# rizar/attention-lvcsr

Hardware: AMD Instinct MI355X
Metric: encoder+attention+decoder training frames/sec (whole node) (higher is better)
Workload: dtype f32; 1 GPU; wsj_base: B=16 utterances x T=800 frames x F=40 fbank per GPU, L=100 labels; 256x256x256x256 BiGRU subsample [1, 1, 2, 2], content_and_conv attention, 256-unit GRU decoder; global_batch=16, per_gpu_batch=16, ragged=False, parallelism=dp1, optimizer=clip100+adadelta+maxnorm1, hip_graph=True, priming_steps=2, encoder_kernels=persistent clusters, full=False

## Files before the change

attention-lvcsr_amd/csrc/gemm.hip:

```cpp
#include "common.h"
#include "lvsr_hip.h"
#include "graph_cache.h"

#define BM 64
#define BN 64
#define BK 16
#define LDS_LD (BM + 4)

struct GemmArgs {
    const float* A; const float* B; float* C; const float* bias;
    int M, N, K, lda, ldb, ldc, transA, transB;
    float alpha, beta;
    int ksplit;
    int kchunk;
    float* part;
    int batch;
    long long sA, sB, sC;
};

__global__ __launch_bounds__(256) void lvsr_sgemm_kernel(GemmArgs g) {
    __shared__ float As[BK][LDS_LD];
    __shared__ float Bs[BK][LDS_LD];
    const int tid = threadIdx.x, lane = tid & 63, wave = tid >> 6;
    const int m0 = blockIdx.y * BM, n0 = blockIdx.x * BN;
    int zsplit = blockIdx.z;
    if (g.batch > 1) {
        g.A += blockIdx.z * g.sA; g.B += blockIdx.z * g.sB; g.C += blockIdx.z * g.sC;
        zsplit = 0;
    }
    const int kbeg = zsplit * g.kchunk;
    const int kend = min(g.K, kbeg + g.kchunk);
    const int rowbase = (wave >> 1) * 32, colbase = (wave & 1) * 32;
    f32x4 acc[2][2];
#pragma unroll
    for (int i = 0; i < 2; ++i)
#pragma unroll
        for (int j = 0; j < 2; ++j) acc[i][j] = (f32x4){0.f, 0.f, 0.f, 0.f};

    for (int k0 = kbeg; k0 < kend; k0 += BK) {
        if (!g.transA) {
            const int kk = tid & 15, mm = tid >> 4;
#pragma unroll
            for (int p = 0; p < 4; ++p) {
                const int m = m0 + mm + p * 16, k = k0 + kk;
                As[kk][mm + p * 16] = (m < g.M && k < kend) ? g.A[(size_t)m * g.lda + k] : 0.f;
            }
        } else {
            const int mm = tid & 63, kk = tid >> 6;
#pragma unroll
            for (int p = 0; p < 4; ++p) {
                const int m = m0 + mm, k = k0 + kk + p * 4;
                As[kk + p * 4][mm] = (m < g.M && k < kend) ? g.A[(size_t)k * g.lda + m] : 0.f;
            }
        }
        if (!g.transB) {
            const int nn = tid & 63, kk = tid >> 6;
#pragma unroll
            for (int p = 0; p < 4; ++p) {
                const int n = n0 + nn, k = k0 + kk + p * 4;
                Bs[kk + p * 4][nn] = (n < g.N && k < kend) ? g.B[(size_t)k * g.ldb + n] : 0.f;
            }
        } else {
            const int kk = tid & 15, nn = tid >> 4;
#pragma unroll
            for (int p = 0; p < 4; ++p) {
                const int n = n0 + nn + p * 16, k = k0 + kk;
                Bs[kk][nn + p * 16] = (n < g.N && k < kend) ? g.B[(size_t)n * g.ldb + k] : 0.f;
            }
        }
        __syncthreads();
#pragma unroll
        for (int ks = 0; ks < BK; ks += 4) {
            const int kr = ks + (lane >> 4), li = lane & 15;
            float a[2], b[2];
            a[0] = As[kr][rowbase + li];
            a[1] = As[kr][rowbase + 16 + li];
            b[0] = Bs[kr][colbase + li];
            b[1] = Bs[kr][colbase + 16 + li];
#pragma unroll
            for (int i = 0; i < 2; ++i)
#pragma unroll
                for (int j = 0; j < 2; ++j)
                    acc[i][j] = __builtin_amdgcn_mfma_f32_16x16x4f32(a[i], b[j], acc[i][j], 0, 0, 0);
        }
        __syncthreads();
    }
#pragma unroll
    for (int i = 0; i < 2; ++i)
#pragma unroll
        for (int j = 0; j < 2; ++j)
#pragma unroll
            for (int r = 0; r < 4; ++r) {
                const int m = m0 + rowbase + i * 16 + (lane >> 4) * 4 + r;
                const int n = n0 + colbase + j * 16 + (lane & 15);
                if (m < g.M && n < g.N) {
                    if (g.ksplit > 1) {
                        g.part[((size_t)zsplit * g.M + m) * g.N + n] = acc[i][j][r];
                    } else {
                        float v = g.alpha * acc[i][j][r];
                        if (g.beta != 0.f) v += g.beta * g.C[(size_t)m * g.ldc + n];
                        if (g.bias) v += g.bias[n];
                        g.C[(size_t)m * g.ldc + n] = v;
                    }
                }
            }
}

typedef float f32x16 __attribute__((ext_vector_type(16)));
#define GM 128
#define GN 128
#define GK 32
#define GLD 36

template <bool CONTIG_K, int TX, bool GUARD>
__device__ __forceinline__ void gemm2_tile_load(const float* __restrict__ p, int ld, int x0, int X, int k0, int kend, bool vec,
                                                float4 (&r)[TX / 32]) {
    if (CONTIG_K) {
#pragma unroll
        for (int h = 0; h < TX / 32; ++h) {
            const int u = threadIdx.x + h * 256;
            const int x = x0 + (u >> 3), k = k0 + (u & 7) * 4;
            if (!GUARD) r[h] = *(const float4*)(p + (size_t)x * ld + k);
            else r[h] = (x < X && k < kend) ? ld4g(p + (size_t)x * ld + k, kend - k, vec) : make_float4(0.f, 0.f, 0.f, 0.f);
        }
    } else {
        const int k = k0 + (threadIdx.x >> 6) * 8 + (threadIdx.x & 7);
#pragma unroll
        for (int h = 0; h < TX / 32; ++h) {
            const int x = x0 + 4 * (h * 8 + ((threadIdx.x >> 3) & 7));
            if (!GUARD) r[h] = *(const float4*)(p + (size_t)k * ld + x);
            else r[h] = (k < kend && x < X) ? ld4g(p + (size_t)k * ld + x, X - x, vec) : make_float4(0.f, 0.f, 0.f, 0.f);
        }
    }
}
__device__ __forceinline__ int gemm2_col(int k) { return (k & ~7) + ((k & 1) << 2) + ((k & 7) >> 1); }

template <bool CONTIG_K, int TX>
__device__ __forceinline__ void gemm2_tile_store(float (*S)[GLD], const float4 (&r)[TX / 32]) {
    if (CONTIG_K) {
#pragma unroll
        for (int h = 0; h < TX / 32; ++h) {
            const int u = threadIdx.x + h * 256;
            const int c0 = ((u & 7) >> 1) * 8 + (u & 1) * 2;
            *(float2*)&S[u >> 3][c0] = make_float2(r[h].x, r[h].z);
            *(float2*)&S[u >> 3][c0 + 4] = make_float2(r[h].y, r[h].w);
        }
    } else {
        const int k = gemm2_col((threadIdx.x >> 6) * 8 + (threadIdx.x & 7));
#pragma unroll
        for (int h = 0; h < TX / 32; ++h) {
            const int x = 4 * (h * 8 + ((threadIdx.x >> 3) & 7));
            S[x][k] = r[h].x; S[x + 1][k] = r[h].y; S[x + 2][k] = r[h].z; S[x + 3][k] = r[h].w;
        }
    }
}

__device__ __forceinline__ int gemm_xcd_order(int L, int total) {
    const int xcd = L & 7, per = total >> 3, rem = total & 7;
    return xcd * per + min(xcd, rem) + (L >> 3);
}

template <int TM, int TN, bool TA, bool TB, bool FAST>
__device__ __forceinline__ void sgemm_tile(GemmArgs g, int bx, int by, int bz) {
    constexpr int MI = TM / 64, NI = TN / 64;
    __shared__ __attribute__((aligned(16))) float As[2][TM][GLD];
    __shared__ __attribute__((aligned(16))) float Bs[2][TN][GLD];
    const int lane = threadIdx.x & 63, wave = threadIdx.x >> 6;
    if (g.batch > 1) {
        g.A += bz * g.sA; g.B += bz * g.sB; g.C += bz * g.sC;
        bz = 0;
    }
    const int m0 = by * TM, n0 = bx * TN;
    const int kbeg = bz * g.kchunk, kend = min(g.K, kbeg + g.kchunk);
    const int wm = (wave >> 1) * (TM / 2), wn = (wave & 1) * (TN / 2);
    const bool vecA = ((g.lda & 3) == 0) && ((((size_t)g.A) & 15) == 0);
    const bool vecB = ((g.ldb & 3) == 0) && ((((size_t)g.B) & 15) == 0);
    f32x16 acc[MI][NI];
#pragma unroll
    for (int i = 0; i < MI; ++i)
#pragma unroll
        for (int j = 0; j < NI; ++j)
#pragma unroll
            for (int r = 0; r < 16; ++r) acc[i][j][r] = 0.f;
    float4 ra[TM / 32], rb[TN / 32];
    const bool inside = FAST && m0 + TM <= g.M && n0 + TN <= g.N;
    if (inside && kbeg + GK <= kend) {
        gemm2_tile_load<!TA, TM, false>(g.A, g.lda, m0, g.M, kbeg, kend, true, ra);
        gemm2_tile_load<TB, TN, false>(g.B, g.ldb, n0, g.N, kbeg, kend, true, rb);
    } else {
        gemm2_tile_load<!TA, TM, true>(g.A, g.lda, m0, g.M, kbeg, kend, vecA, ra);
        gemm2_tile_load<TB, TN, true>(g.B, g.ldb, n0, g.N, kbeg, kend, vecB, rb);
    }
    gemm2_tile_store<!TA, TM>(As[0], ra);
    gemm2_tile_store<TB, TN>(Bs[0], rb);
    __syncthreads();
    int cur = 0;
    const int li = lane & 31, kh = (lane >> 5) * 4;
    for (int k0 = kbeg; k0 < kend; k0 += GK) {
        const bool more = k0 + GK < kend;
        float4 pa[2][MI], pb[2][NI];
#pragma unroll
        for (int i = 0; i < MI; ++i) pa[0][i] = *(const float4*)&As[cur][wm + 32 * i + li][kh];
#pragma unroll
        for (int j = 0; j < NI; ++j) pb[0][j] = *(const float4*)&Bs[cur][wn + 32 * j + li][kh];
#pragma unroll
        for (int q = 0; q < 4; ++q) {
            const int c = q & 1, n = c ^ 1;
            if (q + 1 < 4) {
#pragma unroll
                for (int i = 0; i < MI; ++i) pa[n][i] = *(const float4*)&As[cur][wm + 32 * i + li][kh + 8 * (q + 1)];
#pragma unroll
                for (int j = 0; j < NI; ++j) pb[n][j] = *(const float4*)&Bs[cur][wn + 32 * j + li][kh + 8 * (q + 1)];
            }
            __builtin_amdgcn_sched_barrier(0);
#pragma unroll
            for (int e = 0; e < 4; ++e)
#pragma unroll
                for (int i = 0; i < MI; ++i)
#pragma unroll
                    for (int j = 0; j < NI; ++j) {
                        const float x = e == 0 ? pa[c][i].x : e == 1 ? pa[c][i].y : e == 2 ? pa[c][i].z : pa[c][i].w;
                        const float y = e == 0 ? pb[c][j].x : e == 1 ? pb[c][j].y : e == 2 ? pb[c][j].z : pb[c][j].w;
                        acc[i][j] = __builtin_amdgcn_mfma_f32_32x32x2f32(x, y, acc[i][j], 0, 0, 0);
                    }
            __builtin_amdgcn_sched_barrier(0);
        }
        if (more) {
            if (inside && k0 + 2 * GK <= kend) {
                gemm2_tile_load<!TA, TM, false>(g.A, g.lda, m0, g.M, k0 + GK, kend, true, ra);
                gemm2_tile_load<TB, TN, false>(g.B, g.ldb, n0, g.N, k0 + GK, kend, true, rb);
            } else {
                gemm2_tile_load<!TA, TM, true>(g.A, g.lda, m0, g.M, k0 + GK, kend, vecA, ra);
                gemm2_tile_load<TB, TN, true>(g.B, g.ldb, n0, g.N, k0 + GK, kend, vecB, rb);
            }
            gemm2_tile_store<!TA, TM>(As[cur ^ 1], ra);
            gemm2_tile_store<TB, TN>(Bs[cur ^ 1], rb);
        }
        __syncthreads();
        cur ^= 1;
    }
#pragma unroll
    for (int i = 0; i < MI; ++i)
#pragma unroll
        for (int j = 0; j < NI; ++j)
#pragma unroll
            for (int r = 0; r < 16; ++r) {
                const int m = m0 + wm + i * 32 + (r & 3) + 8 * (r >> 2) + 4 * (lane >> 5);
                const int n = n0 + wn + j * 32 + (lane & 31);
                if (m < g.M && n < g.N) {
                    if (g.ksplit > 1) {
                        g.part[((size_t)bz * g.M + m) * g.N + n] = acc[i][j][r];
                    } else {
                        float v = g.alpha * acc[i][j][r];
                        if (g.beta != 0.f) v += g.beta * g.C[(size_t)m * g.ldc + n];
                        if (g.bias) v += g.bias[n];
                        g.C[(size_t)m * g.ldc + n] = v;
                    }
                }
            }
}
#define GU (GK / 8)
template <bool CONTIG_K, int TX>
__device__ __forceinline__ void gemm1_tile_load(const float* __restrict__ p, int ld, int x0, int X, int k0, int kend, bool vec,
                                               float4 (&r)[TX / 32]) {
#pragma unroll
    for (int h = 0; h < TX / 32; ++h) {
        const int u = threadIdx.x + h * 256;
        float4 v = make_float4(0.f, 0.f, 0.f, 0.f);
        if (CONTIG_K) {
            const int x = x0 + (u % TX), k = k0 + (u / TX) * 4;
            if (x < X && k < kend) v = ld4g(p + (size_t)x * ld + k, kend - k, vec);
        } else {
            const int k = k0 + u / (TX / 4), x = x0 + (u % (TX / 4)) * 4;
            if (k < kend && x < X) v = ld4g(p + (size_t)k * ld + x, X - x, vec);
        }
        r[h] = v;
    }
}
template <bool CONTIG_K, int TX>
__device__ __forceinline__ void gemm1_tile_load_fast(const float* __restrict__ p, int ld, int x0, int k0, float4 (&r)[TX / 32]) {
#pragma unroll
    for (int h = 0; h < TX / 32; ++h) {
        const int u = threadIdx.x + h * 256;
        if (CONTIG_K) r[h] = *(const float4*)(p + (size_t)(x0 + (u % TX)) * ld + k0 + (u / TX) * 4);
        else r[h] = *(const float4*)(p + (size_t)(k0 + u / (TX / 4)) * ld + x0 + (u % (TX / 4)) * 4);
    }
}
template <bool CONTIG_K, int TX>
__device__ __forceinline__ void gemm1_tile_store(float (*S)[TX + 4], const float4 (&r)[TX / 32]) {
#pragma unroll
    for (int h = 0; h < TX / 32; ++h) {
        const int u = threadIdx.x + h * 256;
        if (CONTIG_K) {
            const int x = u % TX, k = (u / TX) * 4;
            S[k + 0][x] = r[h].x; S[k + 1][x] = r[h].y; S[k + 2][x] = r[h].z; S[k + 3][x] = r[h].w;
        } else {
            const int k = u / (TX / 4), x = (u % (TX / 4)) * 4;
            *(float4*)&S[k][x] = r[h];
        }
    }
}

template <int TM, int TN, bool TA, bool TB, bool FAST>
__device__ __forceinline__ void sgemm_tile_kmajor(GemmArgs g, int bx, int by, int bz) {
    constexpr int MI = TM / 64, NI = TN / 64;
    __shared__ __attribute__((aligned(16))) float As[2][GK][TM + 4];
    __shared__ __attribute__((aligned(16))) float Bs[2][GK][TN + 4];
    const int lane = threadIdx.x & 63, wave = threadIdx.x >> 6;
    if (g.batch > 1) {
        g.A += bz * g.sA; g.B += bz * g.sB; g.C += bz * g.sC;
        bz = 0;
    }
    const int m0 = by * TM, n0 = bx * TN;
    const int kbeg = bz * g.kchunk, kend = min(g.K, kbeg + g.kchunk);
    const int wm = (wave >> 1) * (TM / 2), wn = (wave & 1) * (TN / 2);
    const bool vecA = ((g.lda & 3) == 0) && ((((size_t)g.A) & 15) == 0);
    const bool vecB = ((g.ldb & 3) == 0) && ((((size_t)g.B) & 15) == 0);
    f32x16 acc[MI][NI];
#pragma unroll
    for (int i = 0; i < MI; ++i)
#pragma unroll
        for (int j = 0; j < NI; ++j)
#pragma unroll
            for (int r = 0; r < 16; ++r) acc[i][j][r] = 0.f;
    float4 ra[TM / 32], rb[TN / 32];
    const bool inside = FAST && m0 + TM <= g.M && n0 + TN <= g.N;
    if (inside && kbeg + GK <= kend) {
        gemm1_tile_load_fast<!TA, TM>(g.A, g.lda, m0, kbeg, ra);
        gemm1_tile_load_fast<TB, TN>(g.B, g.ldb, n0, kbeg, rb);
    } else {
        gemm1_tile_load<!TA, TM>(g.A, g.lda, m0, g.M, kbeg, kend, vecA, ra);
        gemm1_tile_load<TB, TN>(g.B, g.ldb, n0, g.N, kbeg, kend, vecB, rb);
    }
    gemm1_tile_store<!TA, TM>(As[0], ra);
    gemm1_tile_store<TB, TN>(Bs[0], rb);
    __syncthreads();
    int cur = 0;
    for (int k0 = kbeg; k0 < kend; k0 += GK) {
        const bool more = k0 + GK < kend;
        if (more) {
            if (inside && k0 + 2 * GK <= kend) {
                gemm1_tile_load_fast<!TA, TM>(g.A, g.lda, m0, k0 + GK, ra);
                gemm1_tile_load_fast<TB, TN>(g.B, g.ldb, n0, k0 + GK, rb);
            } else {
                gemm1_tile_load<!TA, TM>(g.A, g.lda, m0, g.M, k0 + GK, kend, vecA, ra);
                gemm1_tile_load<TB, TN>(g.B, g.ldb, n0, g.N, k0 + GK, kend, vecB, rb);
            }
        }
        const int kr0 = lane >> 5, li = lane & 31;
        float pa[2][MI], pb[2][NI];
#pragma unroll
        for (int i = 0; i < MI; ++i) pa[0][i] = As[cur][kr0][wm + 32 * i + li];
#pragma unroll
        for (int j = 0; j < NI; ++j) pb[0][j] = Bs[cur][kr0][wn + 32 * j + li];
#pragma unroll
        for (int s = 0; s < GK / 2; ++s) {
            const int c = s & 1, n = c ^ 1;
            if (s + 1 < GK / 2) {
                const int kr = 2 * (s + 1) + kr0;
#pragma unroll
                for (int i = 0; i < MI; ++i) pa[n][i] = As[cur][kr][wm + 32 * i + li];
#pragma unroll
                for (int j = 0; j < NI; ++j) pb[n][j] = Bs[cur][kr][wn + 32 * j + li];
            }
            __builtin_amdgcn_sched_barrier(0);
#pragma unroll
            for (int i = 0; i < MI; ++i)
#pragma unroll
                for (int j = 0; j < NI; ++j)
                    acc[i][j] = __builtin_amdgcn_mfma_f32_32x32x2f32(pa[c][i], pb[c][j], acc[i][j], 0, 0, 0);
            __builtin_amdgcn_sched_barrier(0);
        }
        if (more) {
            gemm1_tile_store<!TA, TM>(As[cur ^ 1], ra);
            gemm1_tile_store<TB, TN>(Bs[cur ^ 1], rb);
        }
        __syncthreads();
        cur ^= 1;
    }
#pragma unroll
    for (int i = 0; i < MI; ++i)
#pragma unroll
        for (int j = 0; j < NI; ++j)
#pragma unroll
            for (int r = 0; r < 16; ++r) {
                const int m = m0 + wm + i * 32 + (r & 3) + 8 * (r >> 2) + 4 * (lane >> 5);
                const int n = n0 + wn + j * 32 + (lane & 31);
                if (m < g.M && n < g.N) {
                    if (g.ksplit > 1) {
                        g.part[((size_t)bz * g.M + m) * g.N + n] = acc[i][j][r];
                    } else {
                        float v = g.alpha * acc[i][j][r];
                        if (g.beta != 0.f) v += g.beta * g.C[(size_t)m * g.ldc + n];
                        if (g.bias) v += g.bias[n];
                        g.C[(size_t)m * g.ldc + n] = v;
                    }
                }
            }
}
template <bool TA, bool TB, bool FAST>
__device__ __forceinline__ void sgemm128_tile(GemmArgs g, int bx, int by, int bz) { sgemm_tile<128, 128, TA, TB, FAST>(g, bx, by, bz); }

template <bool TA, bool TB, bool FAST>
__global__ __launch_bounds__(256) void lvsr_sgemm64_kernel(GemmArgs g) {
    const int total = gridDim.x * gridDim.y * gridDim.z;
    const int t = gemm_xcd_order(blockIdx.x + gridDim.x * (blockIdx.y + gridDim.y * blockIdx.z), total);
    sgemm_tile_kmajor<64, 64, TA, TB, FAST>(g, t % gridDim.x, (t / gridDim.x) % gridDim.y, t / (gridDim.x * gridDim.y));
}

template <bool TA, bool TB, bool FAST>
__global__ __launch_bounds__(256) void lvsr_sgemm128_kernel(GemmArgs g) {
    const int total = gridDim.x * gridDim.y * gridDim.z;
    const int t = gemm_xcd_order(blockIdx.x + gridDim.x * (blockIdx.y + gridDim.y * blockIdx.z), total);
    sgemm128_tile<TA, TB, FAST>(g, t % gridDim.x, (t / gridDim.x) % gridDim.y, t / (gridDim.x * gridDim.y));
}

#define GROUP_MAX 40
struct GroupDesc {
    const float* A; const float* B; float* C;
    int M, N, K, lda, ldb, ldc;
    float beta;
    int ksplit, kchunk, gx, gy, unit0;
    long long part_off;
};
struct GroupPack { GroupDesc d[GROUP_MAX]; int n, total; float* part; };

template <bool FAST>
__global__ __launch_bounds__(256) void lvsr_sgemm128_grouped_tn_kernel(GroupPack pk) {
    const int t = gemm_xcd_order(blockIdx.x, pk.total);
    int p = 0;
    for (int x = 1; x < pk.n; ++x)
        if (t >= pk.d[x].unit0) p = x;
    const GroupDesc& d = pk.d[p];
    const int local = t - d.unit0;
    GemmArgs g;
    g.A = d.A; g.B = d.B; g.C = d.C; g.bias = nullptr;
    g.M = d.M; g.N = d.N; g.K = d.K; g.lda = d.lda; g.ldb = d.ldb; g.ldc = d.ldc; g.transA = 1; g.transB = 0;
    g.alpha = 1.f; g.beta = d.beta; g.ksplit = d.ksplit; g.kchunk = d.kchunk; g.part = pk.part + d.part_off;
    g.batch = 1; g.sA = g.sB = g.sC = 0;
    sgemm128_tile<true, false, FAST>(g, local % d.gx, (local / d.gx) % d.gy, local / (d.gx * d.gy));
}

__global__ __launch_bounds__(256) void lvsr_sgemm_grouped_reduce(GroupPack pk) {
    const GroupDesc& d = pk.d[blockIdx.y];
    if (d.ksplit <= 1) return;
    const size_t total = (size_t)d.M * d.N;
    const float* part = pk.part + d.part_off;
    for (size_t idx = (size_t)blockIdx.x * 256 + threadIdx.x; idx < total; idx += (size_t)gridDim.x * 256) {
        const int m = (int)(idx / d.N), n = (int)(idx % d.N);
        float s = 0.f;
        for (int z = 0; z < d.ksplit; ++z) s += part[(size_t)z * total + idx];
        if (d.beta != 0.f) s += d.beta * d.C[(size_t)m * d.ldc + n];
        d.C[(size_t)m * d.ldc + n] = s;
    }
}

__global__ __launch_bounds__(256) void lvsr_sgemm_splitk_reduce(GemmArgs g) {
    const size_t total = (size_t)g.M * g.N;
    for (size_t idx = (size_t)blockIdx.x * blockDim.x + threadIdx.x; idx < total; idx += (size_t)gridDim.x * blockDim.x) {
        const int m = (int)(idx / g.N), n = (int)(idx % g.N);
        float s = 0.f;
        for (int z = 0; z < g.ksplit; ++z) s += g.part[(size_t)z * total + idx];
        float v = g.alpha * s;
        if (g.beta != 0.f) v += g.beta * g.C[(size_t)m * g.ldc + n];
        if (g.bias) v += g.bias[n];
        g.C[(size_t)m * g.ldc + n] = v;
    }
}

__global__ __launch_bounds__(256) void lvsr_colsum_kernel(const float* X, int M, int N, int ldx, float* out, float beta,
                                                          int rows_per, float* part) {
    __shared__ float red[4][64];
    const int n = blockIdx.x * 64 + (threadIdx.x & 63);
    const int g = threadIdx.x >> 6;
    const int m0 = blockIdx.y * rows_per, m1 = min(M, m0 + rows_per);
    float s0 = 0.f, s1 = 0.f, s2 = 0.f, s3 = 0.f;
    if (n < N) {
        int m = m0 + g;
        for (; m + 12 < m1; m += 16) {
            s0 += X[(size_t)m * ldx + n];
            s1 += X[(size_t)(m + 4) * ldx + n];
            s2 += X[(size_t)(m + 8) * ldx + n];
            s3 += X[(size_t)(m + 12) * ldx + n];
        }
        for (; m < m1; m += 4) s0 += X[(size_t)m * ldx + n];
    }
    red[g][threadIdx.x & 63] = (s0 + s1) + (s2 + s3);
    __syncthreads();
    if (g == 0 && n < N) {
        const int c = threadIdx.x & 63;
        const float v = ((red[0][c] + red[1][c]) + red[2][c]) + red[3][c];
        if (part) part[(size_t)blockIdx.y * N + n] = v;
        else out[n] = (beta != 0.f ? beta * out[n] : 0.f) + v;
    }
}

#define COLSUM_MANY_MAX 32
struct ColsumMember { const float* X; float* out; float* part; int M, N, ldx, S, rows_per, nx, block0, fin0; float beta; };
struct ColsumPack { ColsumMember m[COLSUM_MANY_MAX]; int n; };
__global__ __launch_bounds__(256) void lvsr_colsum_many_kernel(ColsumPack pk) {
    __shared__ float red[4][64];
    int p = 0;
    for (int i = 1; i < pk.n; ++i)
        if ((int)blockIdx.x >= pk.m[i].block0) p = i;
    const ColsumMember& c = pk.m[p];
    const int local = blockIdx.x - c.block0, bx = local % c.nx, by = local / c.nx;
    const int n = bx * 64 + (threadIdx.x & 63);
    const int g = threadIdx.x >> 6;
    const int m0 = by * c.rows_per, m1 = min(c.M, m0 + c.rows_per);
    const float* X = c.X;
    const int ldx = c.ldx;
    float s0 = 0.f, s1 = 0.f, s2 = 0.f, s3 = 0.f;
    if (n < c.N) {
        int m = m0 + g;
        for (; m + 12 < m1; m += 16) {
            s0 += X[(size_t)m * ldx + n];
            s1 += X[(size_t)(m + 4) * ldx + n];
            s2 += X[(size_t)(m + 8) * ldx + n];
            s3 += X[(size_t)(m + 12) * ldx + n];
        }
        for (; m < m1; m += 4) s0 += X[(size_t)m * ldx + n];
    }
    red[g][threadIdx.x & 63] = (s0 + s1) + (s2 + s3);
    __syncthreads();
    if (g == 0 && n < c.N) {
        const int col = threadIdx.x & 63;
        const float v = ((red[0][col] + red[1][col]) + red[2][col]) + red[3][col];
        if (c.S > 1) c.part[(size_t)by * c.N + n] = v;
        else c.out[n] = (c.beta != 0.f ? c.beta * c.out[n] : 0.f) + v;
    }
}
__global__ __launch_bounds__(256) void lvsr_colsum_many_finish(ColsumPack pk) {
    int p = 0;
    for (int i = 1; i < pk.n; ++i)
        if ((int)blockIdx.x >= pk.m[i].fin0) p = i;
    const ColsumMember& c = pk.m[p];
    if (c.S <= 1) return;
    const int n = ((int)blockIdx.x - c.fin0) * 256 + threadIdx.x;
    if (n >= c.N) return;
    float v = 0.f;
    for (int s = 0; s < c.S; ++s) v += c.part[(size_t)s * c.N + n];
    c.out[n] = (c.beta != 0.f ? c.beta * c.out[n] : 0.f) + v;
}

__global__ __launch_bounds__(256) void lvsr_colsum_finish(const float* part, int S, int N, float* out, float beta) {
    const int n = blockIdx.x * 256 + threadIdx.x;
    if (n >= N) return;
    float v = 0.f;
    for (int s = 0; s < S; ++s) v += part[(size_t)s * N + n];
    out[n] = (beta != 0.f ? beta * out[n] : 0.f) + v;
}

#define COPY_MANY_MAX 32
struct CopyPack { lvsr_copy_desc d[COPY_MANY_MAX]; int n; };
__global__ __launch_bounds__(256) void lvsr_copy2d_many_kernel(CopyPack pk) {
    const lvsr_copy_desc& d = pk.d[blockIdx.y];
    const bool vec = ((d.cols | d.lds | d.ldd) & 3) == 0 && ((((size_t)d.src) | ((size_t)d.dst)) & 15) == 0;
    if (d.rows == 1) {
        for (int c = blockIdx.x * 256 + threadIdx.x; c < d.cols; c += gridDim.x * 256)
            d.dst[c] = d.beta != 0.f ? d.src[c] + d.beta * d.dst[c] : d.src[c];
        return;
    }
    for (int r = blockIdx.x; r < d.rows; r += gridDim.x) {
        const float* s = d.src + (size_t)r * d.lds;
        float* o = d.dst + (size_t)r * d.ldd;
        if (d.beta != 0.f) {
            for (int c = threadIdx.x; c < d.cols; c += 256) o[c] = s[c] + d.beta * o[c];
        } else if (vec) {
            for (int c = threadIdx.x * 4; c < d.cols; c += 1024) *(float4*)(o + c) = *(const float4*)(s + c);
        } else {
            for (int c = threadIdx.x; c < d.cols; c += 256) o[c] = s[c];
        }
    }
}

__global__ __launch_bounds__(256) void lvsr_transpose_kernel(const float* in, int rows, int cols, float* out) {
    __shared__ float tile[32][33];
    const int tx = threadIdx.x & 31, ty = threadIdx.x >> 5;
    const int r0 = blockIdx.y * 32, c0 = blockIdx.x * 32;
    for (int j = ty; j < 32; j += 8) {
        const int r = r0 + j, c = c0 + tx;
        tile[j][tx] = (r < rows && c < cols) ? in[(size_t)r * cols + c] : 0.f;
    }
    __syncthreads();
    for (int j = ty; j < 32; j += 8) {
        const int c = c0 + j, r = r0 + tx;
        if (r < rows && c < cols) out[(size_t)c * rows + r] = tile[tx][j];
    }
}

__global__ __launch_bounds__(256) void lvsr_pack_b_kernel(const float* W, int ldw, int K, int N, int trans, float* P,
                                                          int Kw, int NQ, long long total) {
    for (long long idx = (long long)blockIdx.x * 256 + threadIdx.x; idx < total; idx += (long long)gridDim.x * 256) {
        const int r = (int)(idx & 3), lane = (int)((idx >> 2) & 63);
        const long long g = idx >> 8;
        const int q = (int)(g % NQ), wave = (int)((g / NQ) & 3), tile = (int)(g / NQ / 4);
        const int k = wave * Kw + (lane >> 4) * (Kw >> 2) + 4 * q + r, col = tile * 16 + (lane & 15);
        float v = 0.f;
        if (k < K && col < N) v = trans ? W[(size_t)col * ldw + k] : W[(size_t)k * ldw + col];
        P[idx] = v;
    }
}

extern "C" {

static int sgemm_launch(void* stream, int transA, int transB, int M, int N, int K, float alpha, const float* A, int lda,
                        const float* B, int ldb, float beta, float* C, int ldc, const float* bias, float* ws,
                        long long ws_bytes, int batch, long long sA, long long sB, long long sC) {
    LVSR_REQUIRE(M >= 0 && N >= 0 && K >= 0 && batch >= 1, "lvsr_sgemm: negative dimension");
    if (M == 0 || N == 0) return LVSR_OK;
    GemmArgs g;
    g.batch = batch; g.sA = sA; g.sB = sB; g.sC = sC;
    if (batch > 1) ws = nullptr;
    g.A = A; g.B = B; g.C = C; g.bias = bias;
    g.M = M; g.N = N; g.K = K; g.lda = lda; g.ldb = ldb; g.ldc = ldc; g.transA = transA; g.transB = transB;
    g.alpha = alpha; g.beta = beta; g.ksplit = 1; g.kchunk = 0; g.part = nullptr;
    const bool big = (M >= 96 && N >= 96) || (min(M, N) >= 32 && max(M, N) >= 256 && K >= 2048);
    int tm = big ? GM : BM, tn = big ? GN : BN;
    const int tk = big ? GK : BK;
    int tiles = ((M + tm - 1) / tm) * ((N + tn - 1) / tn);
    const int mid_max = lvsr_knob(LVSR_KNOB_GEMM_MID_TILES) > 0 ? lvsr_knob(LVSR_KNOB_GEMM_MID_TILES) : 2048;
    const bool mid = big && batch == 1 && (tiles < 256 || (tiles < mid_max && K <= 2048));
    if (mid) { tm = 64; tn = 64; tiles = ((M + 63) / 64) * ((N + 63) / 64); }
    g.kchunk = ((K + tk - 1) / tk) * tk;
    if (g.kchunk == 0) g.kchunk = tk;
    const int slots = mid ? 1024 : 512;
    if (ws && 2 * tiles <= slots && K >= 1024) {
        int want = (slots + tiles - 1) / tiles;
        int maxk = K / 256;
        if (want > maxk) want = maxk;
        long long need = (long long)want * M * N * 4;
        while (want > 1 && need > ws_bytes) { --want; need = (long long)want * M * N * 4; }
        if (want > 1) {
            int chunk = (K + want - 1) / want;
            chunk = ((chunk + tk - 1) / tk) * tk;
            g.ksplit = (K + chunk - 1) / chunk;
            g.kchunk = chunk;
            g.part = ws;
        }
    }
    dim3 grid((N + tn - 1) / tn, (M + tm - 1) / tm, batch > 1 ? batch : g.ksplit);
    hipStream_t st = (hipStream_t)stream;
    if (!big) {
        hipLaunchKernelGGL(lvsr_sgemm_kernel, grid, dim3(256), 0, st, g);
    } else {
        const bool fast = (lda & 3) == 0 && (ldb & 3) == 0 && (((size_t)A) & 15) == 0 && (((size_t)B) & 15) == 0 &&
                          (batch == 1 || ((sA & 3) == 0 && (sB & 3) == 0));
#define LVSR_GEMM128(TA_, TB_)                                                                              \
    do {                                                                                                    \
        if (fast) hipLaunchKernelGGL((lvsr_sgemm128_kernel<TA_, TB_, true>), grid, dim3(256), 0, st, g);    \
        else hipLaunchKernelGGL((lvsr_sgemm128_kernel<TA_, TB_, false>), grid, dim3(256), 0, st, g);        \
    } while (0)
#define LVSR_GEMM64(TA_, TB_)                                                                               \
    do {                                                                                                    \
        if (fast) hipLaunchKernelGGL((lvsr_sgemm64_kernel<TA_, TB_, true>), grid, dim3(256), 0, st, g);     \
        else hipLaunchKernelGGL((lvsr_sgemm64_kernel<TA_, TB_, false>), grid, dim3(256), 0, st, g);         \
    } while (0)
        if (mid) {
            if (!transA && !transB) LVSR_GEMM64(false, false);
            else if (transA && !transB) LVSR_GEMM64(true, false);
            else if (!transA && transB) LVSR_GEMM64(false, true);
            else LVSR_GEMM64(true, true);
        } else if (!transA && !transB) LVSR_GEMM128(false, false);
        else if (transA && !transB) LVSR_GEMM128(true, false);
        else if (!transA && transB) LVSR_GEMM128(false, true);
        else LVSR_GEMM128(true, true);
#undef LVSR_GEMM128
#undef LVSR_GEMM64
    }
    if (g.ksplit > 1) {
        int nb = (int)(((size_t)M * N + 255) / 256);
        if (nb > 2048) nb = 2048;
        hipLaunchKernelGGL(lvsr_sgemm_splitk_reduce, dim3(nb), dim3(256), 0, st, g);
    }
    return lvsr_check_launch("lvsr_sgemm");
}

int lvsr_sgemm(void* stream, int transA, int transB, int M, int N, int K, float alpha, const float* A, int lda,
               const float* B, int ldb, float beta, float* C, int ldc, const float* bias, float* ws,
               long long ws_bytes) {
    return sgemm_launch(stream, transA, transB, M, N, K, alpha, A, lda, B, ldb, beta, C, ldc, bias, ws, ws_bytes, 1, 0, 0, 0);
}

int lvsr_sgemm_batched(void* stream, int transA, int transB, int M, int N, int K, float alpha, const float* A, int lda,
                       long long strideA, const float* B, int ldb, long long strideB, float beta, float* C, int ldc,
                       long long strideC, int batch) {
    LVSR_REQUIRE(batch >= 0, "lvsr_sgemm_batched: negative batch");
    if (batch == 0) return LVSR_OK;
    return sgemm_launch(stream, transA, transB, M, N, K, alpha, A, lda, B, ldb, beta, C, ldc, nullptr, nullptr, 0, batch,
                        strideA, strideB, strideC);
}

int lvsr_sgemm_tn_grouped(void* stream, const lvsr_gemm_desc* descs, int n, float* ws, long long ws_bytes) {
    LVSR_REQUIRE(n >= 0 && (n == 0 || descs), "lvsr_sgemm_tn_grouped: bad arguments");
    hipStream_t st = (hipStream_t)stream;
    for (int i = 0; i < n; ++i)
        LVSR_REQUIRE(descs[i].A && descs[i].B && descs[i].C && descs[i].M > 0 && descs[i].N > 0 && descs[i].K > 0,
                     "lvsr_sgemm_tn_grouped: bad descriptor %d", i);
    auto aligned = [](const lvsr_gemm_desc& s) {
        return (s.lda & 3) == 0 && (s.ldb & 3) == 0 && (((size_t)s.A) & 15) == 0 && (((size_t)s.B) & 15) == 0;
    };
    int target = 1024;
    if (ws) {
        for (;; target += 512) {
            long long need = 0;
            bool splits = false;
            for (int i = 0; i < n; ++i) {
                const int want = (descs[i].K + target - 1) / target;
                if (want > 1) { need += (long long)want * descs[i].M * descs[i].N; splits = true; }
            }
            if (!splits || need * 4 <= ws_bytes) break;
        }
    }
    long long off = 0;
    for (int pass = 0; pass < 2; ++pass) {
        GroupPack pk;
        pk.n = 0; pk.part = ws;
        int units = 0;
        bool any_split = false;
        auto launch = [&]() {
            if (pk.n == 0) return;
            pk.total = units;
            if (pass == 0) hipLaunchKernelGGL(lvsr_sgemm128_grouped_tn_kernel<true>, dim3(units), dim3(256), 0, st, pk);
            else hipLaunchKernelGGL(lvsr_sgemm128_grouped_tn_kernel<false>, dim3(units), dim3(256), 0, st, pk);
            if (any_split) hipLaunchKernelGGL(lvsr_sgemm_grouped_reduce, dim3(32, pk.n), dim3(256), 0, st, pk);
            pk.n = 0; units = 0; any_split = false;
        };
        for (int i = 0; i < n; ++i) {
            const lvsr_gemm_desc& s = descs[i];
            if (aligned(s) != (pass == 0)) continue;
            if (pk.n == GROUP_MAX) launch();
            GroupDesc& d = pk.d[pk.n++];
            d.A = s.A; d.B = s.B; d.C = s.C; d.M = s.M; d.N = s.N; d.K = s.K; d.lda = s.lda; d.ldb = s.ldb; d.ldc = s.ldc; d.beta = s.beta;
            d.gx = (s.N + GN - 1) / GN; d.gy = (s.M + GM - 1) / GM;
            int want = ws ? (s.K + target - 1) / target : 1;
            int chunk = (s.K + want - 1) / want;
            chunk = ((chunk + GK - 1) / GK) * GK;
            d.kchunk = chunk;
            d.ksplit = (s.K + chunk - 1) / chunk;
            d.part_off = off;
            if (d.ksplit > 1) { off += (long long)d.ksplit * s.M * s.N; any_split = true; }
            d.unit0 = units;
            units += d.gx * d.gy * d.ksplit;
        }
        launch();
    }
    return lvsr_check_launch("lvsr_sgemm_tn_grouped");
}

int lvsr_colsum(void* stream, const float* X, int M, int N, int ldx, float* out, float beta, float* ws,
                long long ws_bytes) {
    if (N <= 0) return LVSR_OK;
    const int nx = (N + 63) / 64;
    int S = 1;
    if (ws && M >= 512) {
        S = (M + 255) / 256;
        const int want = (1024 + nx - 1) / nx;
        if (S > want) S = want;
        while (S > 1 && (long long)S * N * 4 > ws_bytes) --S;
    }
    const int rows_per = (M + S - 1) / S;
    hipLaunchKernelGGL(lvsr_colsum_kernel, dim3(nx, S), dim3(256), 0, (hipStream_t)stream, X, M, N, ldx, out, beta, rows_per,
                       S > 1 ? ws : nullptr);
    if (S > 1)
        hipLaunchKernelGGL(lvsr_colsum_finish, dim3((N + 255) / 256), dim3(256), 0, (hipStream_t)stream, ws, S, N, out, beta);
    return lvsr_check_launch("lvsr_colsum");
}

int lvsr_colsum_many(void* stream, const lvsr_colsum_desc* descs, int n, float* ws, long long ws_bytes, long long split_ws_bytes) {
    LVSR_REQUIRE(n >= 0 && (n == 0 || descs), "lvsr_colsum_many: bad arguments");
    for (int i = 0; i < n; ++i)
        LVSR_REQUIRE(descs[i].X && descs[i].out && descs[i].M >= 0 && descs[i].N > 0, "lvsr_colsum_many: bad descriptor %d", i);
    for (int i0 = 0; i0 < n; i0 += COLSUM_MANY_MAX) {
        ColsumPack pk;
        pk.n = n - i0 < COLSUM_MANY_MAX ? n - i0 : COLSUM_MANY_MAX;
        int blocks = 0, fin = 0;
        long long off = 0;
        bool any_split = false;
        for (int i = 0; i < pk.n; ++i) {
            const lvsr_colsum_desc& d = descs[i0 + i];
            ColsumMember& c = pk.m[i];
            c.X = d.X; c.out = d.out; c.M = d.M; c.N = d.N; c.ldx = d.ldx; c.beta = d.beta;
            c.nx = (d.N + 63) / 64;
            int S = 1;
            if (ws && d.M >= 512) {
                S = (d.M + 255) / 256;
                const int want = (1024 + c.nx - 1) / c.nx;
                if (S > want) S = want;
                while (S > 1 && (long long)S * d.N * 4 > split_ws_bytes) --S;
            }
            c.S = S;
            c.rows_per = (d.M + S - 1) / S;
            c.part = ws ? ws + off : nullptr;
            if (S > 1) { off += (long long)S * d.N; any_split = true; }
            c.block0 = blocks; blocks += c.nx * S;
            c.fin0 = fin; fin += (d.N + 255) / 256;
        }
        LVSR_REQUIRE(off * 4 <= ws_bytes, "lvsr_colsum_many: workspace too small for the partial sums (%lld bytes needed)", off * 4);
        if (blocks > 0) hipLaunchKernelGGL(lvsr_colsum_many_kernel, dim3(blocks), dim3(256), 0, (hipStream_t)stream, pk);
        if (any_split) hipLaunchKernelGGL(lvsr_colsum_many_finish, dim3(fin), dim3(256), 0, (hipStream_t)stream, pk);
        LVSR_REQUIRE(i0 + COLSUM_MANY_MAX >= n || !any_split, "lvsr_colsum_many: more than %d members with row splits", COLSUM_MANY_MAX);
    }
    return lvsr_check_launch("lvsr_colsum_many");
}

int lvsr_copy2d_many(void* stream, const lvsr_copy_desc* descs, int n) {
    LVSR_REQUIRE(n >= 0 && (n == 0 || descs), "lvsr_copy2d_many: bad arguments");
    for (int i = 0; i < n; ++i)
        LVSR_REQUIRE(descs[i].rows >= 0 && descs[i].cols >= 0 && descs[i].src && descs[i].dst, "lvsr_copy2d_many: bad descriptor %d", i);
    for (int i0 = 0; i0 < n; i0 += COPY_MANY_MAX) {
        CopyPack pk;
        pk.n = n - i0 < COPY_MANY_MAX ? n - i0 : COPY_MANY_MAX;
        for (int i = 0; i < pk.n; ++i) pk.d[i] = descs[i0 + i];
        hipLaunchKernelGGL(lvsr_copy2d_many_kernel, dim3(128, pk.n), dim3(256), 0, (hipStream_t)stream, pk);
    }
    return lvsr_check_launch("lvsr_copy2d_many");
}

int lvsr_transpose(void* stream, const float* in, int rows, int cols, float* out) {
    if (rows <= 0 || cols <= 0) return LVSR_OK;
    hipLaunchKernelGGL(lvsr_transpose_kernel, dim3((cols + 31) / 32, (rows + 31) / 32), dim3(256), 0, (hipStream_t)stream,
                       in, rows, cols, out);
    return lvsr_check_launch("lvsr_transpose");
}

long long lvsr_pack_size(int K, int N) {
    if (K <= 0 || N <= 0) return 0;
    return (long long)((N + 15) / 16) * 16 * 4 * lvsr_pack_kw(K);
}

int lvsr_pack_b(void* stream, const float* W, int ldw, int K, int N, int trans, float* packed) {
    LVSR_REQUIRE(K > 0 && N > 0 && W && packed, "lvsr_pack_b: bad arguments K=%d N=%d", K, N);
    const int Kw = lvsr_pack_kw(K), NQ = Kw / 16;
    const long long total = lvsr_pack_size(K, N);
    int nb = (int)((total + 255) / 256);
    if (nb > 4096) nb = 4096;
    hipLaunchKernelGGL(lvsr_pack_b_kernel, dim3(nb), dim3(256), 0, (hipStream_t)stream, W, ldw, K, N, trans, packed, Kw,
                       NQ, total);
    return lvsr_check_launch("lvsr_pack_b");
}

int lvsr_pack_b_many(void* stream, const lvsr_pack_desc* descs, int n, int use_graph) {
    LVSR_REQUIRE(n >= 0 && (n == 0 || descs), "lvsr_pack_b_many: bad arguments");
    if (n == 0) return LVSR_OK;
    for (int i = 0; i < n; ++i)
        LVSR_REQUIRE(descs[i].K > 0 && descs[i].N > 0 && descs[i].W && descs[i].packed, "lvsr_pack_b_many: bad descriptor %d", i);
    hipStream_t s = (hipStream_t)stream;
    auto enqueue = [&]() {
        for (int i = 0; i < n; ++i) {
            const lvsr_pack_desc& d = descs[i];
            const int Kw = lvsr_pack_kw(d.K), NQ = Kw / 16;
            const long long total = lvsr_pack_size(d.K, d.N);
            int nb = (int)((total + 255) / 256);
            if (nb > 4096) nb = 4096;
            hipLaunchKernelGGL(lvsr_pack_b_kernel, dim3(nb), dim3(256), 0, s, d.W, d.ldw, d.K, d.N, d.trans, d.packed, Kw, NQ, total);
        }
    };
    GraphKey key("pack_many");
    key.add(descs, sizeof(lvsr_pack_desc) * (size_t)n);
    return lvsr_run_graph(s, use_graph, key, enqueue, "lvsr_pack_b_many");
}

}
```

include/lvsr_hip.h:

```cpp
#ifndef LVSR_HIP_H
#define LVSR_HIP_H

#ifdef __cplusplus
extern "C" {
#endif

const char* lvsr_last_error(void);
int lvsr_abi_version(void);
void lvsr_graph_clear(void);
int lvsr_graph_count(void);
void lvsr_graph_suppress(int on);
int lvsr_region_begin(void* stream, const char* key, long long key_bytes);
int lvsr_region_end(void* stream, int keep);
#define LVSR_KNOB_PERSIST_ROWS 0
#define LVSR_KNOB_PERSIST_FLAGS 1
#define LVSR_KNOB_PERSIST_THREADS 2
#define LVSR_KNOB_PHASE_CLOCK 3
#define LVSR_KNOB_MAX_CLUSTER_WGS 4
#define LVSR_KNOB_CLUSTER_RESERVE 5
#define LVSR_KNOB_GEMM_MID_TILES 6
#define LVSR_KNOB_DEC_CLUSTER 7
#define LVSR_KNOB_ENERGY_ROWS 8
#define LVSR_KNOB_COUNT 9
int lvsr_set_knob(int knob, int value);
int lvsr_get_knob(int knob);

int lvsr_sgemm(void* stream, int transA, int transB, int M, int N, int K, float alpha, const float* A, int lda,
               const float* B, int ldb, float beta, float* C, int ldc, const float* bias, float* ws,
               long long ws_bytes);
int lvsr_sgemm_batched(void* stream, int transA, int transB, int M, int N, int K, float alpha, const float* A, int lda,
                       long long strideA, const float* B, int ldb, long long strideB, float beta, float* C, int ldc,
                       long long strideC, int batch);
typedef struct lvsr_gemm_desc {
    const float* A; const float* B; float* C;
    int M, N, K, lda, ldb, ldc;
    float beta;
} lvsr_gemm_desc;
int lvsr_sgemm_tn_grouped(void* stream, const lvsr_gemm_desc* descs, int n, float* ws, long long ws_bytes);
typedef struct lvsr_copy_desc {
    const float* src; float* dst;
    int rows, cols, lds, ldd;
    float beta;
} lvsr_copy_desc;
int lvsr_copy2d_many(void* stream, const lvsr_copy_desc* descs, int n);
int lvsr_colsum(void* stream, const float* X, int M, int N, int ldx, float* out, float beta, float* ws,
                long long ws_bytes);
typedef struct lvsr_colsum_desc {
    const float* X; float* out;
    int M, N, ldx;
    float beta;
} lvsr_colsum_desc;
int lvsr_colsum_many(void* stream, const lvsr_colsum_desc* descs, int n, float* ws, long long ws_bytes, long long split_ws_bytes);
int lvsr_transpose(void* stream, const float* in, int rows, int cols, float* out);

long long lvsr_pack_size(int K, int N);
int lvsr_pack_b(void* stream, const float* W, int ldw, int K, int N, int trans, float* packed);
typedef struct lvsr_pack_desc {
    const float* W;
    float* packed;
    int ldw, K, N, trans;
} lvsr_pack_desc;
int lvsr_pack_b_many(void* stream, const lvsr_pack_desc* descs, int n, int use_graph);

typedef struct lvsr_bigru_fwd_args {
    const float* xg;
    const float* mask;
    const float* Whh_p[2];
    const float* Whg_p[2];
    const float* h0[2];
    float* y;
    float* ysub;
    float* u; float* r; float* c; float* rh;
    int sub, T, B, H;
    int kernel_mask;
    int persistent;
    void* sync_ws;
} lvsr_bigru_fwd_args;
int lvsr_bigru_fwd(void* stream, const lvsr_bigru_fwd_args* a, int use_graph);

typedef struct lvsr_bigru_bwd_args {
    const float* mask; const float* y; const float* u; const float* r; const float* c;
    const float* WhhT_p[2];
    const float* WhgT_p[2];
    const float* h0[2];
    const float* dy;
    float* dxg;
    float* dh_ws;
    float* dh0[2];
    int sub, T, B, H;
    int kernel_mask;
    int persistent;
    void* sync_ws;
} lvsr_bigru_bwd_args;
int lvsr_bigru_bwd(void* stream, const lvsr_bigru_bwd_args* a, int use_graph);
int lvsr_bigru_persist_rows(int B, int H);
long long lvsr_bigru_persist_ws_bytes(int B, int H);

typedef struct lvsr_attdec_args {
    int Tp, B, L, E, D, M, K, c;
    int prior_type;
    int step0;
    int phases;
    int normalizer;
    double p0, p1, p2, p3;
    const float* A; const float* PA; const float* Am;
    long long A_ts, A_bs, PA_ts, PA_bs, Am_ts, Am_bs;
    const float* Ws_p;
    const float* w_e;
    const float* e_bias;
    const float* filters;
    const float* handler;
    const float* Whg_p;
    const float* Whh_p;
    const float* Wdi_p;
    const float* Wdg_p;
    const float* xg;
    const float* ymask;
    float* S;
    float* W;
    float* pos;
    float* WA;
    float* EN;
    float* ZB;
    float* sW;
    float* CV;
    float* U; float* R; float* C; float* RH;
    float* sg;
    float* xin;
    float* ep;
    const int* step_dev;
    int S_ld;
    int label0;
    int group_rows, step_stride;
    const int* group_Tp;
    const int* skip; int skip_stride;
} lvsr_attdec_args;
int lvsr_attdec_fwd(void* stream, const lvsr_attdec_args* a, int use_graph);

typedef struct lvsr_attdec_plain {
    const float* Ws;
    const float* Whg;
    const float* Whh;
    const float* AW;
    int AW_ld;
} lvsr_attdec_plain;
long long lvsr_attdec_persist_ws_bytes(const lvsr_attdec_args* a);
int lvsr_attdec_fwd_persistent(void* stream, const lvsr_attdec_args* a, const lvsr_attdec_plain* w, void* ws, int use_graph);
typedef struct lvsr_attdec_stack2 {
    const float* Whg1; const float* Whh1;
    const float* Ws1;
    const float* F1;
    const float* AW1;
    const float* xg1;
    float* U1; float* R1; float* C1; float* RH1;
    int F1_ld, AW1_ld;
    float* DXG1;
} lvsr_attdec_stack2;
long long lvsr_attdec_stack2_persist_ws_bytes(const lvsr_attdec_args* a);
int lvsr_attdec_fwd_persistent_stack2(void* stream, const lvsr_attdec_args* a, const lvsr_attdec_plain* w,
                                      const lvsr_attdec_stack2* l1, void* ws, int use_graph);
int lvsr_attdec_glimpses(void* stream, const lvsr_attdec_args* a);

typedef struct lvsr_attdec_bwd_args {
    lvsr_attdec_args f;
    const float* WhhT_p;
    const float* WhgT_p;
    const float* WdT_p;
    const float* WsT_p;
    const float* dWA_r;
    const float* dS_r;
    float* DXG;
    float* DWA;
    float* DSW;
    float* DCV;
    float* dPA;
    float* accH;
    float* accWe;
    float* accEb;
    float* ds;
    float* dalp;
    float* dspart; float* dsacc;
    float* Q;
    float* dcvp;
    float* dswp;
    const float* AW;
    const float* QR;
    int AW_ld;
    int ds_ld;
    int parts;
} lvsr_attdec_bwd_args;
int lvsr_attdec_bwd(void* stream, const lvsr_attdec_bwd_args* a, int use_graph);
// ... 182 lines not shown
```

Measured before the change: 1.033 million frames/s.

## Merge aligned/unaligned grouped TN GEMM passes, sort by cost, vectorize split-K reduce

New measurement: 1.045 million frames/s (median of 6 runs). +1.2%, better.

```diff
diff --git a/attention-lvcsr_amd/csrc/gemm.hip b/attention-lvcsr_amd/csrc/gemm.hip
--- a/attention-lvcsr_amd/csrc/gemm.hip
+++ b/attention-lvcsr_amd/csrc/gemm.hip
@@ -1,6 +1,8 @@
 #include "common.h"
 #include "lvsr_hip.h"
 #include "graph_cache.h"
+#include <algorithm>
+#include <vector>
 
 #define BM 64
 #define BN 64
@@ -161,7 +163,7 @@
 }
 
 template <int TM, int TN, bool TA, bool TB, bool FAST>
-__device__ __forceinline__ void sgemm_tile(GemmArgs g, int bx, int by, int bz) {
+__device__ __forceinline__ void sgemm_tile(GemmArgs g, int bx, int by, int bz, bool fast = true) {
     constexpr int MI = TM / 64, NI = TN / 64;
     __shared__ __attribute__((aligned(16))) float As[2][TM][GLD];
     __shared__ __attribute__((aligned(16))) float Bs[2][TN][GLD];
@@ -183,7 +185,7 @@
 #pragma unroll
             for (int r = 0; r < 16; ++r) acc[i][j][r] = 0.f;
     float4 ra[TM / 32], rb[TN / 32];
-    const bool inside = FAST && m0 + TM <= g.M && n0 + TN <= g.N;
+    const bool inside = FAST && fast && m0 + TM <= g.M && n0 + TN <= g.N;
     if (inside && kbeg + GK <= kend) {
         gemm2_tile_load<!TA, TM, false>(g.A, g.lda, m0, g.M, kbeg, kend, true, ra);
         gemm2_tile_load<TB, TN, false>(g.B, g.ldb, n0, g.N, kbeg, kend, true, rb);
@@ -399,7 +401,9 @@
             }
 }
 template <bool TA, bool TB, bool FAST>
-__device__ __forceinline__ void sgemm128_tile(GemmArgs g, int bx, int by, int bz) { sgemm_tile<128, 128, TA, TB, FAST>(g, bx, by, bz); }
+__device__ __forceinline__ void sgemm128_tile(GemmArgs g, int bx, int by, int bz, bool fast = true) {
+    sgemm_tile<128, 128, TA, TB, FAST>(g, bx, by, bz, fast);
+}
 
 template <bool TA, bool TB, bool FAST>
 __global__ __launch_bounds__(256) void lvsr_sgemm64_kernel(GemmArgs g) {
@@ -416,16 +420,19 @@
 }
 
 #define GROUP_MAX 40
+#define FOLD_ELEMS 1024
 struct GroupDesc {
     const float* A; const float* B; float* C;
     int M, N, K, lda, ldb, ldc;
     float beta;
-    int ksplit, kchunk, gx, gy, unit0;
+    int ksplit, kchunk, gx, gy;
+    int unit0;
+    int fast;
+    int fold0;
     long long part_off;
 };
 struct GroupPack { GroupDesc d[GROUP_MAX]; int n, total; float* part; };
 
-template <bool FAST>
 __global__ __launch_bounds__(256) void lvsr_sgemm128_grouped_tn_kernel(GroupPack pk) {
     const int t = gemm_xcd_order(blockIdx.x, pk.total);
     int p = 0;
@@ -438,20 +445,66 @@
     g.M = d.M; g.N = d.N; g.K = d.K; g.lda = d.lda; g.ldb = d.ldb; g.ldc = d.ldc; g.transA = 1; g.transB = 0;
     g.alpha = 1.f; g.beta = d.beta; g.ksplit = d.ksplit; g.kchunk = d.kchunk; g.part = pk.part + d.part_off;
     g.batch = 1; g.sA = g.sB = g.sC = 0;
-    sgemm128_tile<true, false, FAST>(g, local % d.gx, (local / d.gx) % d.gy, local / (d.gx * d.gy));
+    sgemm128_tile<true, false, true>(g, local % d.gx, (local / d.gx) % d.gy, local / (d.gx * d.gy), d.fast != 0);
 }
 
 __global__ __launch_bounds__(256) void lvsr_sgemm_grouped_reduce(GroupPack pk) {
-    const GroupDesc& d = pk.d[blockIdx.y];
-    if (d.ksplit <= 1) return;
+    int p = 0;
+    for (int x = 1; x < pk.n; ++x)
+        if ((int)blockIdx.x >= pk.d[x].fold0) p = x;
+    const GroupDesc& d = pk.d[p];
     const size_t total = (size_t)d.M * d.N;
     const float* part = pk.part + d.part_off;
-    for (size_t idx = (size_t)blockIdx.x * 256 + threadIdx.x; idx < total; idx += (size_t)gridDim.x * 256) {
-        const int m = (int)(idx / d.N), n = (int)(idx % d.N);
-        float s = 0.f;
-        for (int z = 0; z < d.ksplit; ++z) s += part[(size_t)z * total + idx];
-        if (d.beta != 0.f) s += d.beta * d.C[(size_t)m * d.ldc + n];
-        d.C[(size_t)m * d.ldc + n] = s;
+    const size_t base = (size_t)((int)blockIdx.x - d.fold0) * FOLD_ELEMS;
+    const bool vec = (d.N & 3) == 0 && (d.ldc & 3) == 0 && (((size_t)d.C) & 15) == 0 && (((size_t)part) & 15) == 0;
+    size_t idx[4];
+    float s[4] = {0.f, 0.f, 0.f, 0.f};
+#pragma unroll
+    for (int e = 0; e < 4; ++e) idx[e] = vec ? base + 4 * threadIdx.x + e : base + threadIdx.x + 256 * e;
+    int z = 0;
+    if (vec) {
+        if (idx[0] >= total) return;
+        const float* q = part + idx[0];
+        for (; z + 4 <= d.ksplit; z += 4) {
+            float4 v[4];
+#pragma unroll
+            for (int c = 0; c < 4; ++c) v[c] = *(const float4*)(q + (size_t)(z + c) * total);
+#pragma unroll
+            for (int c = 0; c < 4; ++c) { s[0] += v[c].x; s[1] += v[c].y; s[2] += v[c].z; s[3] += v[c].w; }
+        }
+        for (; z < d.ksplit; ++z) {
+            const float4 v = *(const float4*)(q + (size_t)z * total);
+            s[0] += v.x; s[1] += v.y; s[2] += v.z; s[3] += v.w;
+        }
+        float* c = d.C + (idx[0] / d.N) * d.ldc + idx[0] % d.N;
+        if (d.beta != 0.f) {
+            const float4 o = *(const float4*)c;
+            s[0] += d.beta * o.x; s[1] += d.beta * o.y; s[2] += d.beta * o.z; s[3] += d.beta * o.w;
+        }
+        *(float4*)c = make_float4(s[0], s[1], s[2], s[3]);
+        return;
+    }
+    for (; z + 4 <= d.ksplit; z += 4) {
+        float v[4][4];
+#pragma unroll
+        for (int c = 0; c < 4; ++c)
+#pragma unroll
+            for (int e = 0; e < 4; ++e) v[c][e] = idx[e] < total ? part[(size_t)(z + c) * total + idx[e]] : 0.f;
+#pragma unroll
+        for (int c = 0; c < 4; ++c)
+#pragma unroll
+            for (int e = 0; e < 4; ++e) s[e] += v[c][e];
+    }
+    for (; z < d.ksplit; ++z)
+#pragma unroll
+        for (int e = 0; e < 4; ++e) s[e] += idx[e] < total ? part[(size_t)z * total + idx[e]] : 0.f;
+#pragma unroll
+    for (int e = 0; e < 4; ++e) {
+        if (idx[e] >= total) continue;
+        float* c = d.C + (idx[e] / d.N) * d.ldc + idx[e] % d.N;
+        float r = s[e];
+        if (d.beta != 0.f) r += d.beta * *c;
+        *c = r;
     }
 }
 
@@ -691,59 +744,83 @@
                         strideA, strideB, strideC);
 }
 
+static bool group_aligned(const lvsr_gemm_desc& s) {
+    return (s.lda & 3) == 0 && (s.ldb & 3) == 0 && (((size_t)s.A) & 15) == 0 && (((size_t)s.B) & 15) == 0;
+}
+static void group_cut(const lvsr_gemm_desc* s, int n, long long ws_bytes, int* ksplit, int* kchunk) {
+    int target = 1024;
+    if (ws_bytes > 0) {
+        for (;; target += 512) {
+            long long need = 0;
+            bool splits = false;
+            for (int i = 0; i < n; ++i) {
+                const int want = (s[i].K + target - 1) / target;
+                if (want > 1) { need += ((long long)want * s[i].M * s[i].N + 3) / 4 * 4; splits = true; }
+            }
+            if (!splits || need * 4 <= ws_bytes) break;
+        }
+    }
+    for (int i = 0; i < n; ++i) {
+        const int want = ws_bytes > 0 ? (s[i].K + target - 1) / target : 1;
+        int chunk = (s[i].K + want - 1) / want;
+        chunk = ((chunk + GK - 1) / GK) * GK;
+        kchunk[i] = chunk;
+        ksplit[i] = (s[i].K + chunk - 1) / chunk;
+    }
+}
+static void group_order(const lvsr_gemm_desc* s, const int* kchunk, int n, int* order) {
+    for (int i = 0; i < n; ++i) order[i] = i;
+    auto cost = [&](int i) { return (kchunk[i] < s[i].K ? kchunk[i] : s[i].K) * (group_aligned(s[i]) ? 1 : 2); };
+    std::stable_sort(order, order + n, [&](int a, int b) { return cost(a) > cost(b); });
+}
+
+int lvsr_sgemm_tn_grouped_plan(const lvsr_gemm_desc* descs, int n, long long ws_bytes, int* ksplit, int* kchunk) {
+    LVSR_REQUIRE(n >= 0 && (n == 0 || (descs && ksplit && kchunk)), "lvsr_sgemm_tn_grouped_plan: bad arguments");
+    for (int i = 0; i < n; ++i)
+        LVSR_REQUIRE(descs[i].M > 0 && descs[i].N > 0 && descs[i].K > 0, "lvsr_sgemm_tn_grouped_plan: bad descriptor %d", i);
+    group_cut(descs, n, ws_bytes, ksplit, kchunk);
+    return LVSR_OK;
+}
+
 int lvsr_sgemm_tn_grouped(void* stream, const lvsr_gemm_desc* descs, int n, float* ws, long long ws_bytes) {
     LVSR_REQUIRE(n >= 0 && (n == 0 || descs), "lvsr_sgemm_tn_grouped: bad arguments");
     hipStream_t st = (hipStream_t)stream;
     for (int i = 0; i < n; ++i)
         LVSR_REQUIRE(descs[i].A && descs[i].B && descs[i].C && descs[i].M > 0 && descs[i].N > 0 && descs[i].K > 0,
                      "lvsr_sgemm_tn_grouped: bad descriptor %d", i);
-    auto aligned = [](const lvsr_gemm_desc& s) {
-        return (s.lda & 3) == 0 && (s.ldb & 3) == 0 && (((size_t)s.A) & 15) == 0 && (((size_t)s.B) & 15) == 0;
-    };
-    int target = 1024;
-    if (ws) {
-        for (;; target += 512) {
-            long long need = 0;
-            bool splits = false;
-            for (int i = 0; i < n; ++i) {
-                const int want = (descs[i].K + target - 1) / target;
-                if (want > 1) { need += (long long)want * descs[i].M * descs[i].N; splits = true; }
-            }
-            if (!splits || need * 4 <= ws_bytes) break;
-        }
-    }
+    if (!ws || ws_bytes < 0) ws_bytes = 0;
+    std::vector<int> ksplit(n), kchunk(n);
+    group_cut(descs, n, ws_bytes, ksplit.data(), kchunk.data());
     long long off = 0;
-    for (int pass = 0; pass < 2; ++pass) {
+    for (int i0 = 0; i0 < n; i0 += GROUP_MAX) {
+        const int cnt = n - i0 < GROUP_MAX ? n - i0 : GROUP_MAX;
+        int order[GROUP_MAX];
+        group_order(descs + i0, kchunk.data() + i0, cnt, order);
         GroupPack pk;
-        pk.n = 0; pk.part = ws;
-        int units = 0;
-        bool any_split = false;
-        auto launch = [&]() {
-            if (pk.n == 0) return;
-            pk.total = units;
-            if (pass == 0) hipLaunchKernelGGL(lvsr_sgemm128_grouped_tn_kernel<true>, dim3(units), dim3(256), 0, st, pk);
-            else hipLaunchKernelGGL(lvsr_sgemm128_grouped_tn_kernel<false>, dim3(units), dim3(256), 0, st, pk);
-            if (any_split) hipLaunchKernelGGL(lvsr_sgemm_grouped_reduce, dim3(32, pk.n), dim3(256), 0, st, pk);
-            pk.n = 0; units = 0; any_split = false;
-        };
-        for (int i = 0; i < n; ++i) {
+        pk.n = cnt; pk.part = ws;
+        int units = 0, nfold = 0;
+        for (int o = 0; o < cnt; ++o) {
+            const int i = i0 + order[o];
             const lvsr_gemm_desc& s = descs[i];
-            if (aligned(s) != (pass == 0)) continue;
-            if (pk.n == GROUP_MAX) launch();
-            GroupDesc& d = pk.d[pk.n++];
+            GroupDesc& d = pk.d[o];
             d.A = s.A; d.B = s.B; d.C = s.C; d.M = s.M; d.N = s.N; d.K = s.K; d.lda = s.lda; d.ldb = s.ldb; d.ldc = s.ldc; d.beta = s.beta;
             d.gx = (s.N + GN - 1) / GN; d.gy = (s.M + GM - 1) / GM;
-            int want = ws ? (s.K + target - 1) / target : 1;
-            int chunk = (s.K + want - 1) / want;
-            chunk = ((chunk + GK - 1) / GK) * GK;
-            d.kchunk = chunk;
-            d.ksplit = (s.K + chunk - 1) / chunk;
-            d.part_off = off;
-            if (d.ksplit > 1) { off += (long long)d.ksplit * s.M * s.N; any_split = true; }
+            d.ksplit = ksplit[i]; d.kchunk = kchunk[i];
+            d.fast = group_aligned(s) ? 1 : 0;
             d.unit0 = units;
             units += d.gx * d.gy * d.ksplit;
-        }
-        launch();
+            d.fold0 = nfold;
+            d.part_off = off;
+            if (d.ksplit > 1) {
+                const long long mn = (long long)s.M * s.N;
+                off += (d.ksplit * mn + 3) / 4 * 4;
+                nfold += (int)((mn + FOLD_ELEMS - 1) / FOLD_ELEMS);
+            }
+        }
+        LVSR_REQUIRE(off * 4 <= ws_bytes, "lvsr_sgemm_tn_grouped: partials exceed the workspace");
+        pk.total = units;
+        hipLaunchKernelGGL(lvsr_sgemm128_grouped_tn_kernel, dim3(units), dim3(256), 0, st, pk);
+        if (nfold) hipLaunchKernelGGL(lvsr_sgemm_grouped_reduce, dim3(nfold), dim3(256), 0, st, pk);
     }
     return lvsr_check_launch("lvsr_sgemm_tn_grouped");
 }
diff --git a/include/lvsr_hip.h b/include/lvsr_hip.h
--- a/include/lvsr_hip.h
+++ b/include/lvsr_hip.h
@@ -37,6 +37,7 @@
     float beta;
 } lvsr_gemm_desc;
 int lvsr_sgemm_tn_grouped(void* stream, const lvsr_gemm_desc* descs, int n, float* ws, long long ws_bytes);
+int lvsr_sgemm_tn_grouped_plan(const lvsr_gemm_desc* descs, int n, long long ws_bytes, int* ksplit, int* kchunk);
 typedef struct lvsr_copy_desc {
     const float* src; float* dst;
     int rows, cols, lds, ldd;
```
